# UCL-SML/Doubly-Stochastic-DGP

Measured on AMD Instinct MI355X. Metric: ELBO-steps/sec, higher is better.
Workload: dtype f64

## Files before the change

doubly-stochastic-dgp_amd/csrc/head_impl.hpp:

```cpp
#pragma once
#include "chol_lds.hpp"

#define HEAD_THREADS 512
#define HEAD_NW 8
#define HEAD_MAX_N 128
#define HEAD_MAX_DIN 16

static inline size_t head_lds_bytes(int n) { return chol_lds_bytes(n); }
#define HEAD_STAMP(i) do { if (timing && tid == 0) { const long long tn = __builtin_amdgcn_s_memtime(); v.scal[2 + (i)] = (double)(tn - tlast); tlast = tn; } } while (0)
__device__ __forceinline__ void head_factor(const LayerDev& v, const double* __restrict__ theta, double jitter, int white, int timing,
                                            double* dyn) {
  const int n = v.Mp, nb = n >> 4, M = v.M, Din = v.D_in, ld = n + 5;
  lptr W = (lptr)dyn;
  lptr Xd = (lptr)(dyn + n * ld);
  lptr dinv = (lptr)(dyn + n * ld + nb * 16 * 17);
  lptr red = dinv + n;
  gptr Linv = (gptr)v.Linv;
  gptr LinvT = (gptr)v.LinvT;
  __shared__ int s_info;
  const int tid = threadIdx.x, lane = tid & 63, wave = tid >> 6;
  const int g = lane >> 4, c = lane & 15;
  if (tid == 0) s_info = 0;
  long long tlast = timing ? __builtin_amdgcn_s_memtime() : 0;
  const double var = kvar_of(v, theta);
  const double wvar = v.has_white ? softplus_d(theta[v.off_wvar]) + SOFTPLUS_LOWER : 0.0;
  double zreg[HEAD_MAX_N * 16 / HEAD_THREADS];
#pragma unroll
  for (int u = 0; u < HEAD_MAX_N * 16 / HEAD_THREADS; ++u) {
    const int idx = tid + u * HEAD_THREADS, mrow = idx >> 4, d = idx & 15;
    zreg[u] = (mrow < M && d < Din) ? theta[v.off_Z + (int64_t)mrow * Din + d] : 0.0;
  }
  if (tid < 16) red[16 + tid] = (tid < Din) ? 1.0 / (softplus_d(theta[v.off_kls + (v.ard ? tid : 0)]) + SOFTPLUS_LOWER) : 0.0;
  __syncthreads();
#pragma unroll
  for (int u = 0; u < HEAD_MAX_N * 16 / HEAD_THREADS; ++u) {
    const int idx = tid + u * HEAD_THREADS, mrow = idx >> 4, d = idx & 15;
    if (mrow < n) Xd[mrow * 17 + d] = zreg[u] * red[16 + d];
  }
  __syncthreads();
  if (tid < n) {
    double s = 0.0;
#pragma unroll
    for (int d = 0; d < 16; ++d) {
      const double x = Xd[tid * 17 + d];
      s = fma(x, x, s);
    }
    dinv[tid] = s;
  }
  __syncthreads();
  HEAD_STAMP(0);
  {
    gptr R2 = (gptr)v.R2;
    const int npair = nb * (nb + 1) / 2;
    for (int p = wave; p < npair; p += HEAD_NW) {
      int ib = 0;
      while ((ib + 1) * (ib + 2) / 2 <= p) ++ib;
      const int q = p - ib * (ib + 1) / 2;
      d4 G = (d4){0, 0, 0, 0};
      {
        double za[4], zb[4];
#pragma unroll
        for (int s = 0; s < 2; ++s) {
          za[s] = Xd[(16 * ib + c) * 17 + 4 * s + g];
          zb[s] = Xd[(16 * q + c) * 17 + 4 * s + g];
        }
        if (Din > 8) {
#pragma unroll
          for (int s = 2; s < 4; ++s) {
            za[s] = Xd[(16 * ib + c) * 17 + 4 * s + g];
            zb[s] = Xd[(16 * q + c) * 17 + 4 * s + g];
          }
        }
        G = mfma_f64(za[0], zb[0], G);
        G = mfma_f64(za[1], zb[1], G);
        if (Din > 8) {
          G = mfma_f64(za[2], zb[2], G);
          G = mfma_f64(za[3], zb[3], G);
        }
      }
      const int j = 16 * q + c;
      const double nj = dinv[j];
#pragma unroll
      for (int t = 0; t < 4; ++t) {
        const int i = 16 * ib + g + 4 * t;
        double r2 = fmax(dinv[i] + nj - 2.0 * G[t], 0.0);
        if (i == j) r2 = 0.0;
        double k = (i == j) ? 1.0 : 0.0;
        if (i < M && j < M) {
          k = kern_val_rt(v.kern_kind, r2, var);
          if (i == j) k += wvar + jitter;
        }
        W[i * ld + j] = k;
        R2[(int64_t)i * n + j] = r2;
        if (q < ib) R2[(int64_t)j * n + i] = r2;
      }
    }
  }
  __syncthreads();
  HEAD_STAMP(1);

  lds_chol_inverse<true>(W, Xd, n, ld, Linv, LinvT, (int64_t)n, &s_info, timing ? v.scal : nullptr, tlast);
  {
    double s = 0.0;
    for (int i = tid; i < M; i += HEAD_THREADS) s += 2.0 * log(W[i * ld + i]);
    s = sum_wave(s);
    if (lane == 0) red[wave] = s;
  }
  if (white) {
    const int ccol = tid & (HEAD_MAX_N - 1), rgrp = tid >> 7;
    if (ccol < n) {
      gptr Kp = (gptr)v.Kp;
      for (int i = rgrp; i < n; i += HEAD_THREADS / HEAD_MAX_N) Kp[i * n + ccol] = (ccol > i) ? 0.0 : W[i * ld + ccol];
    }
  }
  __syncthreads();
  if (tid == 0) {
    double ldv = 0.0;
    for (int w = 0; w < HEAD_NW; ++w) ldv += red[w];
    v.scal[0] = ldv;
    v.scal[1] = (double)s_info;
  }
  HEAD_STAMP(4);
}

__global__ __launch_bounds__(HEAD_THREADS) void k_head(const double* __restrict__ theta, const LayerDev* __restrict__ layers,
                                                       double* __restrict__ lik_const, int64_t off_lik, int lik_gauss, double jitter,
                                                       int nprep, int keep_kuu, int white, int timing, const HeadRand hr, const HeadGather hg) {
  extern __shared__ __attribute__((aligned(16))) double head_dyn[];
  const int bx = (int)blockIdx.x, l = (int)blockIdx.y;
  if (bx > nprep + hr.nblk) {
    if (l != 0) return;
    const int64_t ct = hg.dx + hg.dy, nth = (int64_t)hg.nblk * HEAD_THREADS;
    for (int64_t i = (int64_t)(bx - 1 - nprep - hr.nblk) * HEAD_THREADS + threadIdx.x; i < hg.n * ct; i += nth) {
      const int64_t r = i / ct, j = i % ct;
      if (j < hg.dx)
        hg.Xd[r * hg.dx + j] = hg.Xs[hg.idx[r] * hg.dx + j];
      else
        hg.Yd[r * hg.dy + (j - hg.dx)] = hg.Ys[hg.idx[r] * hg.dy + (j - hg.dx)];
    }
    return;
  }
  if (bx > nprep) {
    if (hr.count[l] > 0)
      randn_body(hr.seed, (uint64_t)l, hr.count[l], hr.out[l], (int64_t)(bx - 1 - nprep) * HEAD_THREADS + threadIdx.x, (int64_t)hr.nblk * HEAD_THREADS);
    return;
  }
  const LayerDev v = layers[l];
  if (bx > 0)
    prep_body<false>(v, theta, lik_const, off_lik, lik_gauss, bx - 1, nprep);
  else if (!keep_kuu)
    head_factor(v, theta, jitter, white, timing, head_dyn);
}
```

doubly-stochastic-dgp_amd/csrc/linalg.hpp:

```cpp
#pragma once
#include "common.hpp"

struct GemmProblem {
  const double* A;
  const double* B;
  double* C;
  int64_t lda, ldb, ldc, sA, sB, sC;
  int32_t m, n, k;
  int32_t transA, transB;
  int32_t batch, batch_reduce;
  int32_t tiles_m, tiles_n, tile_start;
  double alpha, beta;
  int32_t lower_only;
  int32_t tri;
  const int32_t* order;
  int32_t n_order, pad_order;
};

struct PotrfItem {
  double* W;
  double* Linv;
  double* LinvT;
  double* scal;
  int32_t n, ld, nreal, pad;
  int32_t info_offset, pad2;
};

int gemm_plan(GemmProblem* host, int nprob, int allow_big = 1);
int gemm_plan_lpt(GemmProblem* host, int nprob, std::vector<int32_t>& order, int allow_big = 1);
int gemm_launch(dsdgp_ctx* ctx, const GemmProblem* dev, int nprob, int total_tiles, hipStream_t stream = nullptr);
int pgemm_accum(dsdgp_ctx* ctx, const double* W, int64_t ldw, const double* B, int64_t ldb, double* C, int64_t ldc, int m, int n, int k, double alpha);
int potrf_launch(dsdgp_ctx* ctx, const PotrfItem* dev_items, int nitems, int n_max);
int trtri_launch(dsdgp_ctx* ctx, double* W, double* Linv, int n, int64_t stride, int batch);

struct BigChol {
  int n = 0, batch = 0, nb = 0;
  bool want_inverse = false, from_tri = false;
  double* W = nullptr; double* Linv = nullptr; double* LinvT = nullptr; double* scal = nullptr; double* Tbuf = nullptr;
  int64_t stride = 0, scal_stride = 0;
  bool lookahead = false;
  bool need_factor = true;
  bool xrows = false;
  const double* dinv = nullptr;
  int64_t dinv_stride = 0, dinv_step = 0;
  PotrfItem* diag_items = nullptr;
  std::vector<PotrfItem> items0;
  GemmProblem* gp = nullptr;
  std::vector<int> tiles;
  std::vector<int> nprob, first;
  void* inv_block = nullptr;
  void* dev_block = nullptr;
  void* tbuf_block = nullptr;
};
int bigchol_build(dsdgp_ctx* ctx, BigChol& P, double* W, double* Linv, double* LinvT, double* scal, int batch, int64_t stride,
                  int64_t scal_stride, int n, int nreal, double* Tbuf, bool from_tri, bool need_factor = true);
int bigchol_run(dsdgp_ctx* ctx, const BigChol& P);
void bigchol_free(BigChol& P);

#ifdef __HIPCC__
template <int J, int K>
struct Chol16Upd {
  static __device__ __forceinline__ void run(double (&a)[16], double lij) {
    const double lkj = bcast_lane<K>(lij);
    a[K] -= lij * lkj;
    Chol16Upd<J, K + 1>::run(a, lij);
  }
};
template <int J>
struct Chol16Upd<J, 16> {
  static __device__ __forceinline__ void run(double (&)[16], double) {}
};
template <int J>
struct Chol16 {
  static __device__ __forceinline__ void run(double (&a)[16], int i, double& myinv, int& bad) {
    const double ajj = bcast_lane<J>(a[J]);
    if (!(ajj > 0.0) && bad == 0) bad = J + 1;
    double inv = __builtin_amdgcn_rsq(ajj);
    inv = inv * fma(-0.5 * ajj * inv, inv, 1.5);
    inv = inv * fma(-0.5 * ajj * inv, inv, 1.5);
    myinv = (i == J) ? inv : myinv;
    const double lij = a[J] * inv;
    a[J] = lij;
    Chol16Upd<J, J + 1>::run(a, lij);
    Chol16<J + 1>::run(a, i, myinv, bad);
  }
};
template <>
struct Chol16<16> {
  static __device__ __forceinline__ void run(double (&)[16], int, double&, int&) {}
};

#endif
```

Measured before the change: 1969.

## Specialise head kernel eval, split remainder tiles, lighten barriers, pipeline chol16 pivot

The K_uu tile loop moves into a templated helper that is specialised on kernel kind, so the runtime kernel-type dispatch per element goes away. Leftover tiles are split across pairs of waves by row halves to balance the last round. __syncthreads calls are replaced with lds_barrier. The 16x16 register Cholesky now computes the next pivot's reciprocal sqrt right after updating that column, before the remaining updates, to shorten the dependency chain. It also disables FP contraction on the diagonal jitter add so results stay bit-consistent.

```diff
diff --git a/doubly-stochastic-dgp_amd/csrc/head_impl.hpp b/doubly-stochastic-dgp_amd/csrc/head_impl.hpp
--- a/doubly-stochastic-dgp_amd/csrc/head_impl.hpp
+++ b/doubly-stochastic-dgp_amd/csrc/head_impl.hpp
@@ -7,6 +7,69 @@
 #define HEAD_MAX_DIN 16
 
 static inline size_t head_lds_bytes(int n) { return chol_lds_bytes(n); }
+template <int KIND>
+__device__ __forceinline__ void head_ku(const LayerDev& v, lptr W, lptr Xd, lptr dinv, const int n, const int ld, const double var,
+                                        const double wvar, const double jitter) {
+  const int nb = n >> 4, M = v.M, Din = v.D_in;
+  const int tid = threadIdx.x, lane = tid & 63, wave = tid >> 6;
+  const int g = lane >> 4, c = lane & 15;
+  gptr R2 = (gptr)v.R2;
+  auto tile = [&](int p, int t0, int t1) {
+    int ib = 0;
+    while ((ib + 1) * (ib + 2) / 2 <= p) ++ib;
+    const int q = p - ib * (ib + 1) / 2;
+    d4 G = (d4){0, 0, 0, 0};
+    {
+      double za[4], zb[4];
+#pragma unroll
+      for (int s = 0; s < 2; ++s) {
+        za[s] = Xd[(16 * ib + c) * 17 + 4 * s + g];
+        zb[s] = Xd[(16 * q + c) * 17 + 4 * s + g];
+      }
+      if (Din > 8) {
+#pragma unroll
+        for (int s = 2; s < 4; ++s) {
+          za[s] = Xd[(16 * ib + c) * 17 + 4 * s + g];
+          zb[s] = Xd[(16 * q + c) * 17 + 4 * s + g];
+        }
+      }
+      G = mfma_f64(za[0], zb[0], G);
+      G = mfma_f64(za[1], zb[1], G);
+      if (Din > 8) {
+        G = mfma_f64(za[2], zb[2], G);
+        G = mfma_f64(za[3], zb[3], G);
+      }
+    }
+    const int j = 16 * q + c;
+    const double nj = dinv[j];
+#pragma unroll
+    for (int t = 0; t < 4; ++t) {
+      if (t < t0 || t >= t1) continue;
+      const int i = 16 * ib + g + 4 * t;
+      double r2 = fmax(dinv[i] + nj - 2.0 * G[t], 0.0);
+      if (i == j) r2 = 0.0;
+      double k = (i == j) ? 1.0 : 0.0;
+      if (i < M && j < M) {
+        k = kern_val<KIND>(r2, var);
+        if (i == j) {
+#pragma clang fp contract(off)
+          k += wvar + jitter;
+        }
+      }
+      W[i * ld + j] = k;
+      R2[(int64_t)i * n + j] = r2;
+      if (q < ib) R2[(int64_t)j * n + i] = r2;
+    }
+  };
+  const int npair = nb * (nb + 1) / 2, nfull = npair / HEAD_NW * HEAD_NW, rem = npair - nfull;
+  for (int p = wave; p < nfull; p += HEAD_NW) tile(p, 0, 4);
+  if (2 * rem <= HEAD_NW) {
+    if (wave < 2 * rem) tile(nfull + (wave >> 1), 2 * (wave & 1), 2 * (wave & 1) + 2);
+  } else if (wave < rem) {
+    tile(nfull + wave, 0, 4);
+  }
+}
+
 #define HEAD_STAMP(i) do { if (timing && tid == 0) { const long long tn = __builtin_amdgcn_s_memtime(); v.scal[2 + (i)] = (double)(tn - tlast); tlast = tn; } } while (0)
 __device__ __forceinline__ void head_factor(const LayerDev& v, const double* __restrict__ theta, double jitter, int white, int timing,
                                             double* dyn) {
@@ -31,13 +94,13 @@
     zreg[u] = (mrow < M && d < Din) ? theta[v.off_Z + (int64_t)mrow * Din + d] : 0.0;
   }
   if (tid < 16) red[16 + tid] = (tid < Din) ? 1.0 / (softplus_d(theta[v.off_kls + (v.ard ? tid : 0)]) + SOFTPLUS_LOWER) : 0.0;
-  __syncthreads();
+  lds_barrier();
 #pragma unroll
   for (int u = 0; u < HEAD_MAX_N * 16 / HEAD_THREADS; ++u) {
     const int idx = tid + u * HEAD_THREADS, mrow = idx >> 4, d = idx & 15;
     if (mrow < n) Xd[mrow * 17 + d] = zreg[u] * red[16 + d];
   }
-  __syncthreads();
+  lds_barrier();
   if (tid < n) {
     double s = 0.0;
 #pragma unroll
@@ -47,56 +110,13 @@
     }
     dinv[tid] = s;
   }
-  __syncthreads();
+  lds_barrier();
   HEAD_STAMP(0);
-  {
-    gptr R2 = (gptr)v.R2;
-    const int npair = nb * (nb + 1) / 2;
-    for (int p = wave; p < npair; p += HEAD_NW) {
-      int ib = 0;
-      while ((ib + 1) * (ib + 2) / 2 <= p) ++ib;
-      const int q = p - ib * (ib + 1) / 2;
-      d4 G = (d4){0, 0, 0, 0};
-      {
-        double za[4], zb[4];
-#pragma unroll
-        for (int s = 0; s < 2; ++s) {
-          za[s] = Xd[(16 * ib + c) * 17 + 4 * s + g];
-          zb[s] = Xd[(16 * q + c) * 17 + 4 * s + g];
-        }
-        if (Din > 8) {
-#pragma unroll
-          for (int s = 2; s < 4; ++s) {
-            za[s] = Xd[(16 * ib + c) * 17 + 4 * s + g];
-            zb[s] = Xd[(16 * q + c) * 17 + 4 * s + g];
-          }
-        }
-        G = mfma_f64(za[0], zb[0], G);
-        G = mfma_f64(za[1], zb[1], G);
-        if (Din > 8) {
-          G = mfma_f64(za[2], zb[2], G);
-          G = mfma_f64(za[3], zb[3], G);
-        }
-      }
-      const int j = 16 * q + c;
-      const double nj = dinv[j];
-#pragma unroll
-      for (int t = 0; t < 4; ++t) {
-        const int i = 16 * ib + g + 4 * t;
-        double r2 = fmax(dinv[i] + nj - 2.0 * G[t], 0.0);
-        if (i == j) r2 = 0.0;
-        double k = (i == j) ? 1.0 : 0.0;
-        if (i < M && j < M) {
-          k = kern_val_rt(v.kern_kind, r2, var);
-          if (i == j) k += wvar + jitter;
-        }
-        W[i * ld + j] = k;
-        R2[(int64_t)i * n + j] = r2;
-        if (q < ib) R2[(int64_t)j * n + i] = r2;
-      }
-    }
-  }
-  __syncthreads();
+  if (v.kern_kind == DSDGP_KERN_RBF)
+    head_ku<DSDGP_KERN_RBF>(v, W, Xd, dinv, n, ld, var, wvar, jitter);
+  else
+    head_ku<DSDGP_KERN_MATERN52>(v, W, Xd, dinv, n, ld, var, wvar, jitter);
+  lds_barrier();
   HEAD_STAMP(1);
 
   lds_chol_inverse<true>(W, Xd, n, ld, Linv, LinvT, (int64_t)n, &s_info, timing ? v.scal : nullptr, tlast);
@@ -113,7 +133,7 @@
       for (int i = rgrp; i < n; i += HEAD_THREADS / HEAD_MAX_N) Kp[i * n + ccol] = (ccol > i) ? 0.0 : W[i * ld + ccol];
     }
   }
-  __syncthreads();
+  lds_barrier();
   if (tid == 0) {
     double ldv = 0.0;
     for (int w = 0; w < HEAD_NW; ++w) ldv += red[w];
diff --git a/doubly-stochastic-dgp_amd/csrc/linalg.hpp b/doubly-stochastic-dgp_amd/csrc/linalg.hpp
--- a/doubly-stochastic-dgp_amd/csrc/linalg.hpp
+++ b/doubly-stochastic-dgp_amd/csrc/linalg.hpp
@@ -71,23 +71,38 @@
   static __device__ __forceinline__ void run(double (&)[16], double) {}
 };
 template <int J>
-struct Chol16 {
-  static __device__ __forceinline__ void run(double (&a)[16], int i, double& myinv, int& bad) {
-    const double ajj = bcast_lane<J>(a[J]);
-    if (!(ajj > 0.0) && bad == 0) bad = J + 1;
-    double inv = __builtin_amdgcn_rsq(ajj);
-    inv = inv * fma(-0.5 * ajj * inv, inv, 1.5);
-    inv = inv * fma(-0.5 * ajj * inv, inv, 1.5);
+__device__ __forceinline__ double chol16_pivot_inv(const double (&a)[16], int& bad) {
+  const double ajj = bcast_lane<J>(a[J]);
+  if (!(ajj > 0.0) && bad == 0) bad = J + 1;
+  double inv = __builtin_amdgcn_rsq(ajj);
+  inv = inv * fma(-0.5 * ajj * inv, inv, 1.5);
+  inv = inv * fma(-0.5 * ajj * inv, inv, 1.5);
+  return inv;
+}
+template <int J>
+struct Chol16Step {
+  static __device__ __forceinline__ void run(double (&a)[16], int i, double& myinv, int& bad, double inv) {
     myinv = (i == J) ? inv : myinv;
     const double lij = a[J] * inv;
     a[J] = lij;
-    Chol16Upd<J, J + 1>::run(a, lij);
-    Chol16<J + 1>::run(a, i, myinv, bad);
+    if constexpr (J + 1 < 16) {
+      {
+        const double lkj = bcast_lane<J + 1>(lij);
+        a[J + 1] -= lij * lkj;
+      }
+      const double inv1 = chol16_pivot_inv<J + 1>(a, bad);
+      Chol16Upd<J, J + 2>::run(a, lij);
+      Chol16Step<J + 1>::run(a, i, myinv, bad, inv1);
+    }
   }
 };
+template <int J>
+struct Chol16;
 template <>
-struct Chol16<16> {
-  static __device__ __forceinline__ void run(double (&)[16], int, double&, int&) {}
+struct Chol16<0> {
+  static __device__ __forceinline__ void run(double (&a)[16], int i, double& myinv, int& bad) {
+    Chol16Step<0>::run(a, i, myinv, bad, chol16_pivot_inv<0>(a, bad));
+  }
 };
 
 #endif
```

Result: no change. 1967 (median of 3 runs) (-0.1%).
